# KdaiP/StableTTS

Hardware: AMD Instinct MI355X
Metric: mel-frames/sec (whole node), 31M DiT, n_timesteps=10+CFG (higher is better)
Workload: dtype f16

## Files before the change

stabletts_amd/csrc/attention.hip:

```cpp
#include "common.h"
#include "launch.h"

#if (defined(ST_ABL_NOEXP) || defined(ST_ABL_NOSUM)) && !defined(ST_DEVTOOLS)
#error "ST_ABL_* (ablation builds: results are garbage) need -DST_DEVTOOLS"
#endif
#ifdef ST_ABL_NOEXP
constexpr bool kAblNoExp = true;
#else
constexpr bool kAblNoExp = false;
#endif
#ifdef ST_ABL_NOSUM
constexpr bool kAblNoSum = true;
#else
constexpr bool kAblNoSum = false;
#endif
#ifndef ST_ATTN_WAVES
#define ST_ATTN_WAVES 8
#endif

namespace st {

template <class P, bool TRAIN, bool SPLIT = false, bool VLO = false>
__global__ __launch_bounds__(64 * ST_ATTN_WAVES, ST_ATTN_WAVES >= 16 || SPLIT ? 2 : 4) void attention_kernel(const AttnArgs a) {
    static_assert(!(TRAIN && SPLIT), "split-precision scores: inference kernel only");
    static_assert(!VLO || (TRAIN && !SPLIT), "hi + lo v: training kernel only");
    constexpr bool X3 = SPLIT || VLO;
    constexpr int NW = ST_ATTN_WAVES, QB = 32 * NW, QTILE = QB;
    using vec8 = typename P::vec8;
    constexpr int TILE_BYTES = 64 * 128;
    constexpr int NBUF = 3;
    constexpr int NT = X3 ? 3 : 2;
    constexpr int SMEM = NT * NBUF * TILE_BYTES > NW * 32 * 144 ? NT * NBUF * TILE_BYTES : NW * 32 * 144;
    __shared__ __attribute__((aligned(16))) unsigned char smem[SMEM];
    __shared__ float wave_lse[NW];
    unsigned char* Ks = smem;
    unsigned char* Vs = smem + NBUF * TILE_BYTES;
    unsigned char* KLs = smem + 2 * NBUF * TILE_BYTES;
    unsigned char* VLs = KLs;

    const int T = a.T, Tp = a.Tp, H = a.H;
    const int qtiles = (T + QB - 1) / QB;
    const int j = blockIdx.x >> 3;
    const int qt = j % qtiles, nh = (j / qtiles) * 8 + (blockIdx.x & 7);
    if (nh >= a.n_items * H) return;
    const int n = nh / H, h = nh % H;
    const int mb = n % a.mask_mod;
    if (a.t_lim && qt * QTILE >= a.t_lim[mb]) return;
    const int kvend = a.kv_end[mb];
    const int nfull = a.n_full[mb];
    const float* kbias = a.kbias + (size_t)mb * Tp;

    const int tid = threadIdx.x, lane = tid & 63;
    const int wave = __builtin_amdgcn_readfirstlane(tid >> 6);
    const int l31 = lane & 31, hi = lane >> 5;
    const int query = qt * QB + wave * 32 + l31;

    const unsigned char* qbase = (const unsigned char*)a.q + ((size_t)nh * T) * 128;
    const unsigned char* kbase = (const unsigned char*)a.k + ((size_t)nh * T) * 128;
    const unsigned char* vbase = (const unsigned char*)a.vt + ((size_t)nh * 64) * Tp * 2;
    const unsigned char* qlbase = SPLIT ? (const unsigned char*)a.q_lo + ((size_t)nh * T) * 128 : nullptr;
    const unsigned char* klbase = SPLIT ? (const unsigned char*)a.k_lo + ((size_t)nh * T) * 128 : nullptr;
    const unsigned char* vlbase = VLO ? (const unsigned char*)a.vt_lo + ((size_t)nh * 64) * Tp * 2 : nullptr;
    if constexpr (TRAIN) {
        if (qt * QB >= kvend) {
            if (query < T) {
                unsigned char* orow = (unsigned char*)a.out + (((size_t)n * T + query) * (H * 64) + h * 64) * 2 + hi * 64;
#pragma unroll
                for (int i = 0; i < 4; ++i) *(uint4*)(orow + 16 * i) = make_uint4(0, 0, 0, 0);
                if (hi == 0) a.lse[(size_t)nh * T + query] = 0.f;
            }
            return;
        }
    }

    vec8 qf[4];
#pragma unroll
    for (int ks = 0; ks < 4; ++ks) {
        uint4 v = make_uint4(0, 0, 0, 0);
        if (query < T) v = *(const uint4*)(qbase + (size_t)query * 128 + ks * 32 + hi * 16);
        qf[ks] = as_vec8<P>(v);
    }
    vec8 qlf[SPLIT ? 4 : 1];
    if constexpr (SPLIT) {
#pragma unroll
        for (int ks = 0; ks < 4; ++ks) {
            uint4 v = make_uint4(0, 0, 0, 0);
            if (query < T) v = *(const uint4*)(qlbase + (size_t)query * 128 + ks * 32 + hi * 16);
            qlf[ks] = as_vec8<P>(v);
        }
    }

    const int ntiles = (kvend + 63) >> 6;
    auto sgpr_ptr = [](const unsigned char* p) {
        const uintptr_t v = (uintptr_t)p;
        return (const unsigned char*)(((uintptr_t)(unsigned)__builtin_amdgcn_readfirstlane((int)(v >> 32)) << 32) |
                                      (unsigned)__builtin_amdgcn_readfirstlane((int)(unsigned)v));
    };
    auto issueKV = [&](int kt, int buf) {
        auto k_piece = [&](int piece) {
            int ln = lane;
            if constexpr (TRAIN) asm volatile("" : "+v"(ln));
            const int row = piece * 8 + (ln >> 3);
            const int seg = (ln & 7) ^ ((row >> 1) & 7);
            const int key = min(kt * 64 + row, T - 1);
            glds16s(sgpr_ptr(kbase), (unsigned)(key * 128 + seg * 16), Ks + buf * TILE_BYTES + piece * 1024);
            if constexpr (SPLIT) glds16s(sgpr_ptr(klbase), (unsigned)(key * 128 + seg * 16), KLs + buf * TILE_BYTES + piece * 1024);
        };
        auto v_piece = [&](int piece) {
            const int row = piece * 8 + (lane >> 3);
            const int seg = (lane & 7) ^ ((row >> 1) & 7);
            glds16s(sgpr_ptr(vbase + (size_t)kt * 128), (unsigned)((row * Tp + seg * 8) * 2), Vs + buf * TILE_BYTES + piece * 1024);
            if constexpr (VLO) glds16s(sgpr_ptr(vlbase + (size_t)kt * 128), (unsigned)((row * Tp + seg * 8) * 2), VLs + buf * TILE_BYTES + piece * 1024);
        };
        if constexpr (NW <= 8) {
#pragma unroll
            for (int k = 0; k < 8 / NW; ++k) { k_piece(wave * (8 / NW) + k); v_piece(wave * (8 / NW) + k); }
        } else {
            if (wave < 8) k_piece(wave); else v_piece(wave - 8);
        }
    };

    int row_off[2], swz[2];
#pragma unroll
    for (int b = 0; b < 2; ++b) {
        const int row = b * 32 + l31;
        row_off[b] = row * 128; swz[b] = (row >> 1) & 7;
    }

    f32x16_t o[2];
#pragma unroll
    for (int d = 0; d < 2; ++d)
#pragma unroll
        for (int r = 0; r < 16; ++r) o[d][r] = 0.f;
    constexpr float kBig = 8192.0f, kLazyTrain = 8.0f, kFloor = -20000.0f;
    unsigned drop_rh = 0;
    if constexpr (TRAIN) { if (a.drop.thresh16) drop_rh = a.drop.rowh[(size_t)nh * T + (query < T ? query : T - 1)]; }
    float m_ref = 0.f, l_run = 0.f;
    vec8 qaug, kaug;
#pragma unroll
    for (int i = 0; i < 8; ++i) { qaug[i] = to16<P>(0.f); kaug[i] = to16<P>(0.f); }
    if (hi == 0) kaug[0] = to16<P>(1.0f);

    if (ntiles > 0) issueKV(0, 0);
    if (ntiles > 1) { issueKV(1, 1); if constexpr (NW <= 8) { if constexpr (NW == 8) { if constexpr (X3) ST_DMA_WAIT(3); else ST_DMA_WAIT(2); } else { if constexpr (X3) ST_DMA_WAIT(6); else ST_DMA_WAIT(4); } } else ST_DMA_WAIT(1); }
    else ST_DMA_WAIT(0);
    __syncthreads();

    const int ntiles_run = ntiles;
    bool dead = false;
    if constexpr (!TRAIN) dead = a.t_lim && qt * QB + wave * 32 >= a.t_lim[mb];
    int buf = 0;
    for (int kt = 0; kt < ntiles_run; ++kt) {
        if (kt + 2 < ntiles_run) issueKV(kt + 2, buf >= 1 ? buf - 1 : NBUF - 1);
        if (!dead) {

        f32x16_t s[2];
        const bool partial = (kt + 1) * 64 > nfull;
        auto scores = [&]() __attribute__((always_inline)) {
#pragma unroll
            for (int kb = 0; kb < 2; ++kb) {
#pragma unroll
                for (int r = 0; r < 16; ++r) s[kb][r] = 0.f;
                s[kb] = P::mfma(kaug, qaug, s[kb]);
                const unsigned char* kp = Ks + buf * TILE_BYTES + row_off[kb];
#pragma unroll
                for (int ks = 0; ks < 4; ++ks) {
                    const vec8 kfrag = as_vec8<P>(*(const uint4*)(kp + (((ks * 2 + hi) ^ swz[kb]) << 4)));
                    s[kb] = P::mfma(kfrag, qf[ks], s[kb]);
                    if constexpr (SPLIT) {
                        s[kb] = P::mfma(kfrag, qlf[ks], s[kb]);
                        const unsigned char* klp = KLs + buf * TILE_BYTES + row_off[kb];
                        s[kb] = P::mfma(as_vec8<P>(*(const uint4*)(klp + (((ks * 2 + hi) ^ swz[kb]) << 4))), qf[ks], s[kb]);
                    }
                }
                __builtin_amdgcn_sched_barrier(0);
            }
            if (partial) {
#pragma unroll
                for (int kb = 0; kb < 2; ++kb)
#pragma unroll
                    for (int g4 = 0; g4 < 4; ++g4) {
                        const float4 bz = *(const float4*)(kbias + kt * 64 + kb * 32 + 8 * g4 + 4 * hi);
                        s[kb][4 * g4 + 0] += bz.x; s[kb][4 * g4 + 1] += bz.y;
                        s[kb][4 * g4 + 2] += bz.z; s[kb][4 * g4 + 3] += bz.w;
                    }
            }
        };
        vec8 pf[4];
        float psum[2];
        scores();
        if constexpr (TRAIN) {
            float mx = s[0][0];
#pragma unroll
            for (int kb = 0; kb < 2; ++kb)
#pragma unroll
                for (int r = 0; r < 16; ++r) mx = fmaxf(mx, s[kb][r]);
            mx = xor32_max(mx);
// ... 313 lines not shown
        }
    }
}

template <class P>
static hipError_t launch_attention_small(const AttnArgs& a, hipStream_t s) {
    static bool attr_done_dev[64] = {};
    int dev_ = 0;
    if (hipGetDevice(&dev_) != hipSuccess || dev_ < 0 || dev_ >= 64) return hipErrorInvalidDevice;
    if (!attr_done_dev[dev_]) {
        hipError_t e = hipFuncSetAttribute((const void*)attention_small_kernel<P>, hipFuncAttributeMaxDynamicSharedMemorySize, kAttnSmallLds);
        if (e != hipSuccess) return e;
        attr_done_dev[dev_] = true;
    }
    const int total = a.n_items * a.H * ((a.T + 31) / 32);
    const int grid = ((total + 7) / 8) * 8;
    hipLaunchKernelGGL((attention_small_kernel<P>), dim3(grid), dim3(512), kAttnSmallLds, s, a);
    return hipGetLastError();
}

hipError_t launch_attention(int dtype, const AttnArgs& a, hipStream_t s) {
    if (!a.zeros || !a.kbias) return hipErrorInvalidValue;
    const int qtiles = (a.T + 32 * ST_ATTN_WAVES - 1) / (32 * ST_ATTN_WAVES);
    const int total = a.n_items * a.H * qtiles;
    if (!a.lse && !a.q_lo && a.small_max_blocks > 0 && total <= a.small_max_blocks)
        return dtype == DT_BF16 ? launch_attention_small<OpBF16>(a, s) : launch_attention_small<OpF16>(a, s);
    const int grid = 8 * ((a.n_items * a.H + 7) / 8) * qtiles;
    if (a.lse) {
        if (a.vt_lo) {
            if (dtype == DT_BF16) hipLaunchKernelGGL((attention_kernel<OpBF16, true, false, true>), dim3(grid), dim3(64 * ST_ATTN_WAVES), 0, s, a);
            else                  hipLaunchKernelGGL((attention_kernel<OpF16, true, false, true>), dim3(grid), dim3(64 * ST_ATTN_WAVES), 0, s, a);
            return hipGetLastError();
        }
        if (dtype == DT_BF16) hipLaunchKernelGGL((attention_kernel<OpBF16, true>), dim3(grid), dim3(64 * ST_ATTN_WAVES), 0, s, a);
        else                  hipLaunchKernelGGL((attention_kernel<OpF16, true>), dim3(grid), dim3(64 * ST_ATTN_WAVES), 0, s, a);
        return hipGetLastError();
    }
    if (a.q_lo || a.k_lo) {
        if (!a.q_lo || !a.k_lo) return hipErrorInvalidValue;
        static bool attr_done_dev[64][2] = {};
        int dev_ = 0;
        if (hipGetDevice(&dev_) != hipSuccess || dev_ < 0 || dev_ >= 64) return hipErrorInvalidDevice;
        const int di = dtype == DT_BF16 ? 0 : 1;
        const void* fn = di == 0 ? (const void*)attention_kernel<OpBF16, false, true> : (const void*)attention_kernel<OpF16, false, true>;
        if (!attr_done_dev[dev_][di]) {
            hipError_t e = hipFuncSetAttribute(fn, hipFuncAttributeMaxDynamicSharedMemorySize, 0);
            (void)e;
            attr_done_dev[dev_][di] = true;
        }
        if (di == 0) hipLaunchKernelGGL((attention_kernel<OpBF16, false, true>), dim3(grid), dim3(64 * ST_ATTN_WAVES), 0, s, a);
        else         hipLaunchKernelGGL((attention_kernel<OpF16, false, true>), dim3(grid), dim3(64 * ST_ATTN_WAVES), 0, s, a);
        return hipGetLastError();
    }
    if (dtype == DT_BF16) hipLaunchKernelGGL((attention_kernel<OpBF16, false>), dim3(grid), dim3(64 * ST_ATTN_WAVES), 0, s, a);
    else                  hipLaunchKernelGGL((attention_kernel<OpF16, false>), dim3(grid), dim3(64 * ST_ATTN_WAVES), 0, s, a);
    return hipGetLastError();
}

}
```

stabletts_amd/csrc/engine.cpp:

```cpp
#include "engine_dit.h"
#include "train_launch.h"
#include "mas_launch.h"
#include "align_train_launch.h"

#include <algorithm>
#include <cmath>
#include <cstdio>
#include <cstring>
#include <map>
#include <string>
#include <vector>

using namespace st;
using namespace sthost;

namespace sthost {
std::string g_create_error;

const char* kProfNames[PC_COUNT] = {
    "prep", "prenet_conv", "in_proj", "film_ln1", "qkv_rope", "attention", "out_proj", "ln2",
    "ffn_conv1", "ffn_conv2", "lsc_conv", "final_proj", "ode_update", "train_forward", "train_backward"};

int dev_alloc(st_engine* e, void** p, size_t bytes) {
    HIPCHK(e, hipMalloc(p, bytes ? bytes : 16));
// ... 371 lines not shown
    };
    if (film) {
        ConvGemmArgs a = base_args(e, p, dit->inx, N);
        a.a0 = p.x16; a.c0 = dit->Mp; a.a0_mod = p.B; a.a1 = p.x16lo; a.c1 = dit->Mp; a.a1_mod = p.B; a.c2 = dit->Mp;
        a.bias = nullptr;
        a.add32 = p.cpart; a.add_clamp = p.B;
        a.out32 = p.X; a.out16 = p.skip16[0];
        fuse_ln1(a, 0);
        ProfScope ps(e, s, PC_INPROJ, conv_flops(p, dit->inx, N));
        HIPCHK(e, gemm(e, 1, EPI_F32, a, s));
    } else {
        FilmLnArgs a; memset(&a, 0, sizeof(a));
        a.X = p.X; a.h16 = p.h16; a.film = nullptr; a.film_mod = 1;
        a.ada = ada_of(0); a.ada_stride = 6 * C; a.shift_off = 0; a.scale_off = C;
        a.mask = mask; a.mask_mod = p.B; a.mask_out = 0; a.T = T; a.rows = N * T;
        ProfScope ps(e, s, PC_FILM_LN1, 0);
        HIPCHK(e, launch_film_ln(e->dt, a, s));
    }
    if (film && cap) capture(e, "h0", p.skip16[0], rowsC, true, s);
    for (int i = 0; i < L; ++i) {
        const std::string bn = "b" + std::to_string(i) + ".";
        const float* ada_i = ada_of(i);
        if (skips && i >= L / 2) {
            const int j = i - L / 2;
            ConvGemmArgs a = base_args(e, p, dit->lsc[j], N);
            a.a0 = p.cur16; a.c0 = C; a.a1 = p.skip16[L - 1 - i]; a.c1 = C;
            a.out32 = p.X;
            fuse_ln1(a, i);
            ProfScope ps(e, s, PC_LSC, conv_flops(p, dit->lsc[j], N));
            if (!(dit->skip_mask >> PC_LSC & 1)) HIPCHK(e, gemm(e, 3, EPI_F32, a, s));
        }
        if (cap) { capture(e, bn + "x1", p.X, rowsC, false, s); capture(e, bn + "h1", p.h16, rowsC, true, s); }
        {
            ConvGemmArgs a = base_args(e, p, dit->qkv[i], N);
            a.a0 = p.h16; a.c0 = C;
            a.q = p.q16; a.k = p.k16; a.vt = p.vt16; a.rope_cos = dit->rope_cos; a.rope_sin = dit->rope_sin;
            if (split_qk) { a.q_lo = p.q16lo; a.k_lo = p.k16lo; }
            a.Tp = p.Tp; a.n_heads = dit->H;
            if ((int)dit->qkv_frag.size() == L) a.w_frag = dit->qkv_frag[i];
            a.qscale = 1.4426950408889634f / sqrtf((float)(C / dit->H));
            ProfScope ps(e, s, PC_QKV, conv_flops(p, dit->qkv[i], N));
            if (!(dit->skip_mask >> PC_QKV & 1)) HIPCHK(e, gemm(e, 1, EPI_QKV, a, s));
        }
        if (cap) {
            capture(e, bn + "q", p.q16, rowsC, true, s); capture(e, bn + "k", p.k16, rowsC, true, s);
            capture(e, bn + "vt", p.vt16, (int64_t)N * C * p.Tp, true, s);
        }
        {
            AttnArgs a; memset(&a, 0, sizeof(a));
            a.q = p.q16; a.k = p.k16; a.vt = p.vt16; a.out = p.ao16; a.kbias = p.kbias; a.mask_mod = p.B; a.zeros = e->zeros;
            a.kv_end = p.kv_end; a.n_full = p.n_full; a.T = T; a.Tp = p.Tp; a.H = dit->H; a.n_items = N;
            a.small_max_blocks = dit->conc == 1 ? dit->attn_small_blocks : 0;
            if (split_qk) { a.q_lo = p.q16lo; a.k_lo = p.k16lo; }
            if (dec_fast_paths) a.lse_max = dit->lse_cells;
            if (ragged) a.t_lim = p.t_lim;
            ProfScope ps(e, s, PC_ATTN, 4.0 * (double)N * dit->H * (double)T * T * (C / dit->H));
            if (!(dit->skip_mask >> PC_ATTN & 1)) HIPCHK(e, launch_attention(e->dt, a, s));
        }
        if (cap) capture(e, bn + "attn", p.ao16, rowsC, true, s);
        const bool fused = dec_fast_paths && dit->fused_ffn && !cap && (int)dit->ffn_stream.size() == L && dit->ffn_stream[i] &&
                           (int64_t)dit->conc * N * ((T + kFfnFusedFrames - 1) / kFfnFusedFrames) >= e->tile.big_min_blocks;
        void* h2buf = fused ? p.h2_16 : p.h16;
        {
            ConvGemmArgs a = base_args(e, p, dit->oproj[i], N);
            a.a0 = p.ao16; a.c0 = C; a.mask = mask; a.gate = ada_i + 2 * C; a.gate_stride = 6 * C; a.out32 = p.X;
            a.ln_h16 = h2buf; a.ln_film = nullptr; a.ln_film_mod = 1;
            a.ln_ada = ada_i; a.ln_ada_stride = 6 * C; a.ln_shift_off = 3 * C; a.ln_scale_off = 4 * C; a.ln_mask_out = 1;
            if (dec_fast_paths && (int)dit->oproj_frag.size() == L && !cap) a.w_frag = dit->oproj_frag[i];
            ProfScope ps(e, s, PC_OPROJ, conv_flops(p, dit->oproj[i], N));
            if (!(dit->skip_mask >> PC_OPROJ & 1)) HIPCHK(e, gemm(e, 1, EPI_RESGATE, a, s));
        }
        if (cap) { capture(e, bn + "x2", p.X, rowsC, false, s); capture(e, bn + "h2", p.h16, rowsC, true, s); }
        if (!fused) {
            ConvGemmArgs a = base_args(e, p, dit->ffn1[i], N);
            a.a0 = p.h16; a.c0 = C; a.mask = mask; a.flags = GF_SILU | GF_MASK; a.out16 = p.u16;
            ProfScope ps(e, s, PC_FFN1, conv_flops(p, dit->ffn1[i], N));
            HIPCHK(e, gemm(e, 3, EPI_ACT16, a, s));
        }
        if (cap) capture(e, bn + "u", p.u16, (int64_t)N * T * F, true, s);
        void* copy16 = (skips && i + 1 < L / 2) ? p.skip16[i + 1] : p.cur16;
        {
            ConvGemmArgs a = base_args(e, p, dit->ffn2[i], N);
            a.a0 = p.u16; a.c0 = F; a.mask = mask; a.gate = ada_i + 5 * C; a.gate_stride = 6 * C; a.out32 = p.X;
            if (fused) { a.a0 = h2buf; a.c0 = C; a.w = dit->ffn_stream[i]; a.bias1 = dit->ffn1[i].bias; a.cmid = F; a.flags = GF_SILU | GF_MASK; }
            a.out16 = copy16;
            if (i + 1 == L) a.out16_lo = p.cur16lo;
            if (i + 1 < ln1_by_ffn) fuse_ln1(a, i + 1);
            else if (dec_fast_paths && !cap) a.out32_readonly = 1;
            ProfScope ps(e, s, PC_FFN2, conv_flops(p, dit->ffn2[i], N) + (fused ? conv_flops(p, dit->ffn1[i], N) : 0.0));
            if (dit->skip_mask >> PC_FFN2 & 1) {}
            else if (fused && dit->fused_ffn == 3) HIPCHK(e, launch_ffn_wino_f16(a, s));
            else if (fused) HIPCHK(e, e->dt == DT_BF16 ? launch_ffn_fused_bf16(a, s) : launch_ffn_fused_f16(a, s));
            else HIPCHK(e, gemm(e, 3, EPI_RESGATE, a, s));
        }
        if (cap) {
            if (film && i + 1 < ln1_by_ffn) capture(e, bn + "x3", copy16, rowsC, true, s);
            else capture(e, bn + "x3", p.X, rowsC, false, s);
        }
    }
    {
        ConvGemmArgs a = base_args(e, p, dit->fin, N);
        a.a0 = p.cur16; a.c0 = C; a.a1 = p.cur16lo; a.c1 = C; a.c2 = C; a.mask = mask; a.flags = GF_MASK; a.out32 = p.v32;
        ProfScope ps(e, s, PC_FINAL, conv_flops(p, dit->fin, N));
        HIPCHK(e, gemm(e, 1, EPI_F32, a, s));
    }
    if (cap) capture(e, "v", p.v32, (int64_t)N * T * dit->Mp, false, s);
// ... 566 lines not shown
    HIPCHK(e, hipStreamSynchronize((hipStream_t)stream));
    *nonfinite = *dit->status_host != 0;
    dit->arena_poisoned(e);
    return ST_OK;
}

int st_cfm_loss_prep(const float* x1, const float* z, const float* t_rand, float sigma_min, int B, int M, int T, float* t, float* y,
                     float* u, void* stream) {
    if (!x1 || !z || !t_rand || !t || !y || !u) return align_fail(ST_ERR_INVALID, "null tensor pointer");
    if (B < 1 || M < 1 || T < 1 || B > 65535) return align_fail(ST_ERR_INVALID, "shape out of range");
    if (launch_cfm_loss_prep(x1, z, t_rand, sigma_min, B, M, T, t, y, u, (hipStream_t)stream) != hipSuccess)
        return align_fail(ST_ERR_HIP, "cfm_loss_prep kernel launch failed");
    return ST_OK;
}

int st_cfm_loss(const float* pred, const float* u, const float* mask, int B, int M, int T, float* scratch, float* loss, void* stream) {
    if (!pred || !u || !mask || !scratch || !loss) return align_fail(ST_ERR_INVALID, "null tensor pointer");
    if (B < 1 || M < 1 || T < 1) return align_fail(ST_ERR_INVALID, "shape out of range");
    if (launch_cfm_loss(pred, u, mask, B, M, T, scratch, loss, (hipStream_t)stream) != hipSuccess)
        return align_fail(ST_ERR_HIP, "cfm_loss kernel launch failed");
    return ST_OK;
}

int st_cfm_loss_backward(const float* pred, const float* u, const float* scratch, const float* grad_loss, int B, int M, int T,
                         float* grad_pred, void* stream) {
    if (!pred || !u || !scratch || !grad_loss || !grad_pred) return align_fail(ST_ERR_INVALID, "null tensor pointer");
    if (B < 1 || M < 1 || T < 1) return align_fail(ST_ERR_INVALID, "shape out of range");
    if (launch_cfm_loss_bwd(pred, u, scratch, grad_loss, B, M, T, grad_pred, (hipStream_t)stream) != hipSuccess)
        return align_fail(ST_ERR_HIP, "cfm_loss_bwd kernel launch failed");
    return ST_OK;
}

int st_cfm_loss_scratch_floats(void) { return 2 * kCfmLossBlocks + 2; }

int st_last_solve_stats(const st_engine* e, int64_t* nfe, int64_t* steps, int64_t* rejects) {
    if (!e) return ST_ERR_INVALID;
    const DitState* dit = dit_or_null(e);
    if (nfe) *nfe = dit ? dit->last_nfe : 0;
    if (steps) *steps = dit ? dit->last_steps : 0;
    if (rejects) *rejects = dit ? dit->last_rejects : 0;
    return ST_OK;
}

int st_set_option(st_engine* e, const char* name, int value) {
    if (!e || !name) return ST_ERR_INVALID;
    const std::string n(name);
    if (n == "attention_precision") {
        if (value != 0 && value != 1) return e->fail(ST_ERR_INVALID, "attention_precision: 0 (16-bit q / k operands) or 1 (split hi + lo operands)");
        if (e->kind != KIND_DECODER) return e->fail(ST_ERR_UNSUPPORTED, "attention_precision: CFM decoder handles only");
        DitState* dit = dit_of(e);
        if (value != dit->attn_split) { dit->drop_graphs(); dit->attn_split = value; }
        return ST_OK;
    }
    if (n == "fused_ffn") return e->fail(ST_ERR_INVALID, "fused_ffn is read-only (ST_FUSED_FFN at st_create)");
    return e->fail(ST_ERR_INVALID, std::string("unknown option: ") + name);
}

int st_get_option(const st_engine* e, const char* name, int* value) {
    if (!e || !name || !value) return ST_ERR_INVALID;
    const DitState* dit = dit_or_null(e);
    const std::string n(name);
    if (n == "attention_precision") { *value = dit ? dit->attn_split : 0; return ST_OK; }
    if (n == "fused_ffn") { *value = dit ? dit->fused_ffn : -1; return ST_OK; }
    return ST_ERR_INVALID;
}

int st_attention_stats(st_engine* e, void* stream, float* max_lse) {
    if (!e || !max_lse) return ST_ERR_INVALID;
    DitState* dit = dit_or_null(e);
    if (!dit || !dit->lse_cells) return e->fail(ST_ERR_STATE, "attention statistics unavailable (allocation failed at st_create)");
    HIPCHK(e, hipSetDevice(e->device));
    HIPCHK(e, hipStreamSynchronize((hipStream_t)stream));
    int cells[kLseCells * 16];
    HIPCHK(e, hipMemcpy(cells, dit->lse_cells, sizeof(cells), hipMemcpyDeviceToHost));
    int best = (int)0x80000000;
    for (int c = 0; c < kLseCells; ++c) best = std::max(best, cells[c * 16]);
    HIPCHK(e, hipMemsetD32((hipDeviceptr_t)dit->lse_cells, (int)0x80000000, kLseCells * 16));
    if (best == (int)0x80000000) { *max_lse = -INFINITY; return ST_OK; }
    const int bits = best >= 0 ? best : best ^ 0x7fffffff;
    float v; memcpy(&v, &bits, 4);
    *max_lse = v * 0.6931471805599453f;
    return ST_OK;
}

int st_debug_capture(st_engine* e, int enable) {
    if (!e) return ST_ERR_INVALID;
    e->capture = enable != 0;
    if (!enable) {
        hipSetDevice(e->device);
        hipDeviceSynchronize();
        for (auto& kv : e->caps) if (kv.second.dev) hipFree(kv.second.dev);
        e->caps.clear();
    }
    return ST_OK;
}

int64_t st_debug_fetch(st_engine* e, const char* name, float* host_out, int64_t capacity) {
    if (!e || !name) return ST_ERR_INVALID;
    auto it = e->caps.find(name);
    if (it == e->caps.end() || !it->second.dev) { e->err = std::string("no captured tensor named ") + name; return ST_ERR_INVALID; }
    Captured& c = it->second;
    if (!host_out) return c.n;
    if (capacity < c.n) { e->err = "capacity too small"; return ST_ERR_INVALID; }
    if (hipSetDevice(e->device) != hipSuccess || hipDeviceSynchronize() != hipSuccess) return ST_ERR_HIP;
    if (!c.is16) {
        if (hipMemcpy(host_out, c.dev, (size_t)c.n * 4, hipMemcpyDeviceToHost) != hipSuccess) return ST_ERR_HIP;
        return c.n;
    }
    float* tmp = nullptr;
    if (hipMalloc((void**)&tmp, (size_t)c.n * 4) != hipSuccess) return ST_ERR_HIP;
    hipError_t r = launch_cvt16_to_f32(e->dt, c.dev, tmp, c.n, nullptr);
    if (r == hipSuccess) r = hipMemcpy(host_out, tmp, (size_t)c.n * 4, hipMemcpyDeviceToHost);
    hipFree(tmp);
    return r == hipSuccess ? c.n : (int64_t)ST_ERR_HIP;
}
// ... 47 lines not shown
```

stabletts_amd/csrc/engine_dit.h:

```cpp
#pragma once
#include "engine_internal.h"
#include "stream_fork.h"

constexpr int kMaxParts = 1 + sthost::StreamFork::kMaxChildren;
constexpr size_t kSplitKBytes = 32u << 20;

namespace sthost {

struct TrainState;

struct DitState : KindState {
    st_config cfg{};
    bool dec = true;
    int M = 0, Mp = 0, C = 0, F = 0, H = 0, L = 0, K = 0, G = 0;
    int n_vocab = 0;
    std::string blk(int i) const { return dec ? "blocks." + std::to_string(i) + ".block." : "encoder." + std::to_string(i) + "."; }
    struct PackList { std::vector<st::PackJob> jobs; st::PackJob* dev = nullptr; unsigned nblocks = 0; bool ready = false; bool recording = false; };
    PackList pk_fwd, pk_T;
    bool packed_once = false;

    std::vector<Conv> pre;
    Conv inx, inc, fin;
    std::vector<Conv> lsc, qkv, oproj, ffn1, ffn2;
    std::vector<void*> oproj_frag;
    std::vector<void*> qkv_frag;
    std::vector<void*> ffn_stream;

    float* rope_cos = nullptr; float* rope_sin = nullptr; int rope_T = 0;
    void* sink = nullptr;

    int64_t last_nfe = 0, last_steps = 0, last_rejects = 0;
    int* status_host = nullptr; int* status_dev = nullptr;
    bool arena_poisoned(st_engine* e) { if (status_host && *status_host) { *status_host = 0; e->ws_sig = 0; return true; } return false; }

    void* adams_buf = nullptr; size_t adams_bytes = 0;
    unsigned skip_mask = 0;
    int qkv_ws_min_tiles = 400;
    int qkv_ws = 1;
    int oproj_ws = 1;
    int oproj_ws_min_tiles = 1000;
    int qkv_rc1 = 1;
    int fused_ffn = -1;
    int attn_split = 0;
    unsigned* lse_cells = nullptr;
    int attn_small_blocks = 32;
    int conc = 1;
    StreamFork part_streams;

    struct SolveGraph {
        int B, T, n_steps, solver, use_cfg; float cfg_strength; const char* ws; int parts; int seen; hipGraphExec_t exec;
    };
    std::vector<SolveGraph> graphs;
    hipStream_t gstream = nullptr;
    void drop_graphs() {
        for (auto& g : graphs) if (g.exec) hipGraphExecDestroy(g.exec);
        graphs.clear();
    }

    TrainState* train = nullptr;

    ~DitState() override;
    int finalize(st_engine* e) override;
    int repack(st_engine* e, hipStream_t s) override;
    int64_t device_bytes() const override;
    int64_t train_serial() const override;
    void params_moved() override { pk_fwd.ready = false; pk_T.ready = false; drop_graphs(); }
    void arena_moved() override { drop_graphs(); }
};

inline DitState* dit_of(st_engine* e) { return state_of<DitState>(e); }
inline const DitState* dit_of(const st_engine* e) { return state_of<DitState>(e); }
inline const DitState* dit_or_null(const st_engine* e) { return e->kind == KIND_DECODER || e->kind == KIND_TEXT_ENCODER ? dit_of(e) : nullptr; }
inline DitState* dit_or_null(st_engine* e) { return const_cast<DitState*>(dit_or_null(const_cast<const st_engine*>(e))); }

int arena_fresh(st_engine* e, uint64_t sig, size_t used_bytes, hipStream_t s);
int ensure_rope(st_engine* e, int T, hipStream_t s);
int check_ready(st_engine* e, Kind kind, int B, int T);
int pack_all(st_engine* e, hipStream_t s);
bool pk_replay(st_engine* e, DitState::PackList& L, hipStream_t s, int* rc);
void pk_begin(DitState::PackList& L);
int pk_end(st_engine* e, DitState::PackList& L, hipStream_t s);
int pk_weight(st_engine* e, DitState::PackList& L, const float* src, int cout, int cin_total, int K, int ci_off, int ci_cnt, void* dst,
              int row_off, int cin_p, int col_off, int slice_w, int lo, hipStream_t s);
int pk_weight_t(st_engine* e, DitState::PackList& L, const float* src, int cout, int cin_total, int taps, int ci_off, int ci_cnt, void* dst,
                int cin_p, int ld, int col_off, hipStream_t s);
int pk_copy(st_engine* e, DitState::PackList& L, float* dst, const float* src, int n, hipStream_t s);

struct Plan {
    int B, T, Tp, N, Pn, n_t;
    bool cfg;
    void *mu16, *pre1, *pre2, *cond16, *cond16lo, *x16, *x16lo, *h16, *h2_16, *q16, *k16, *q16lo, *k16lo, *vt16, *ao16, *u16, *cur16, *cur16lo;
    void* skip16[8];
    float *cpart, *X, *v32, *xstate, *kbuf[7], *ynew, *ode_partial, *ode_out, *tvals, *emb, *th, *tau, *film, *cvec, *ada, *ada_tmp;
    int *n_full, *kv_end;
    int* t_lim;
    float* kbias;
    float* maskbuf;
// ... 18 lines not shown
```

stabletts_amd/csrc/launch.h:

```cpp
#pragma once
#include <hip/hip_runtime.h>
#include <stdint.h>

namespace st {

enum { DT_BF16 = 0, DT_F16 = 1 };

enum { EPI_ACT16 = 0, EPI_F32 = 1, EPI_RESGATE = 2, EPI_QKV = 3,
       EPI_GELU16 = 4,
       EPI_SILU = 5 };
enum { GF_SILU = 1, GF_MASK = 2,
       GF_K2_V_ONLY = 4 };

struct ConvGemmArgs {
    const void* a0; const void* a1;
    int c0, c1;
    int c2;
    int a0_mod, a1_mod;
    const void* w;
    long long w_item_stride;
    const float* bias;
    int cout, T, n_items;
    int tiles_f, tiles_c;
    const float* mask; int mask_mod;
// ... 11 lines not shown
    const float* rope_cos; const float* rope_sin;
    int Tp; float qscale; int n_heads;
    const void* zeros;
    const void* w_frag;
    void* sink;
    void* ln_h16;
    const float* ln_film; int ln_film_stride; int ln_film_mod;
    const float* ln_ada; int ln_ada_stride; int ln_shift_off; int ln_scale_off;
    int ln_mask_out;
    const int* t_lim; int t_lim_mod;
    void* act16; const void* dact16;
    unsigned long long drop_seed; unsigned drop_thresh16; float drop_scale;
    int ksplit;
    const float* bias1; int cmid;
    unsigned long long* dbg;
};

enum { G2_T128 = 0, G2_RC = 1, G2_K3PIPE = 2,
       G2_BIG = 3,
       G2_T64 = 4, G2_RC64 = 5,
       G2_PHASED = 6,
       G2_RC1 = 7 };
hipError_t launch_conv_gemm2_bf16(int cfg, int taps, int epi, const ConvGemmArgs& a, hipStream_t s);
hipError_t launch_conv_gemm2_f16(int cfg, int taps, int epi, const ConvGemmArgs& a, hipStream_t s);
hipError_t launch_splitk_finish_bf16(int epi, const ConvGemmArgs& a, const float* part, int S, hipStream_t s);
hipError_t launch_splitk_finish_f16(int epi, const ConvGemmArgs& a, const float* part, int S, hipStream_t s);
constexpr int kFfnFusedFrames = 126;
hipError_t launch_ffn_fused_bf16(const ConvGemmArgs& a, hipStream_t s);
hipError_t launch_ffn_fused_f16(const ConvGemmArgs& a, hipStream_t s);
hipError_t launch_pack_ffn_stream(int dtype, const float* src, int stage, int F, void* dst, hipStream_t s);
hipError_t launch_pack_ffn_wino(const float* src, int stage, int F, void* dst, hipStream_t s);
hipError_t launch_ffn_wino_f16(const ConvGemmArgs& a, hipStream_t s);
hipError_t launch_qkv_ws(int dtype, const ConvGemmArgs& a, hipStream_t s);
hipError_t launch_oproj_ws(int dtype, const ConvGemmArgs& a, hipStream_t s);
hipError_t launch_pack_qkv_frag(int dtype, const float* src, int plane, void* dst, hipStream_t s);
constexpr int kGemmFramesPerTile = 128;
constexpr int kGemmChannelsPerTile = 128;

struct DropCfg { unsigned long long seed; unsigned thresh16; float scale; const unsigned* rowh; const unsigned* colh; };

struct AttnArgs {
    const void* q; const void* k; const void* vt; void* out;
    const void* q_lo; const void* k_lo;
    const void* vt_lo;
    unsigned* lse_max;
    const float* kbias; int mask_mod;
    const int* kv_end; const int* n_full;
    int T, Tp, H, n_items;
    const void* zeros;
    float* lse;
    DropCfg drop;
    const int* t_lim;
    int small_max_blocks;
};
constexpr int kLseCells = 16;
hipError_t launch_attention(int dtype, const AttnArgs& a, hipStream_t s);

struct FilmLnArgs {
    float* X;
    void* h16;
    const float* film; int film_stride; int film_mod;
    const float* ada; int ada_stride;
    int shift_off, scale_off;
    const float* mask; int mask_mod;
    int mask_out;
    int T, rows;
};
hipError_t launch_film_ln(int dtype, const FilmLnArgs& a, hipStream_t s);

hipError_t launch_time_embed(const float* t, int n_t, int dim, float* emb, hipStream_t s);
hipError_t launch_silu_rows(const float* in, int64_t n, float* out, hipStream_t s);
struct LinearJobs { const float* in[8]; const float* W[8]; const float* bias[8]; float* out[8]; int n; };
hipError_t launch_linear_multi(const LinearJobs& J, int n, int k, int o, int silu_in, int silu_out, hipStream_t s);
hipError_t launch_linear(const float* in, int n, int k, const float* W, const float* bias, int o,
                         float* out, int silu_in, int silu_out, hipStream_t s);
constexpr int kFrameHalo = 4;
hipError_t launch_mask_prep(const float* mask, int B, int T, int Tp, int* n_full, int* kv_end, float* kbias, int* t_lim, hipStream_t s);

hipError_t launch_to_time_major(int dtype, const float* in, int B, int C, int T, int Cp,
                                float* out32, void* out16, void* out16lo, hipStream_t s);
hipError_t launch_from_time_major(const float* in, int B, int C, int T, int Cp, float* out, hipStream_t s, int* nonfinite = nullptr);
hipError_t launch_embed_tokens(const long long* tokens, const long long* lengths, const float* emb, int n_vocab,
                               int C, float scale, int B, int T, float* X, float* mask_out, hipStream_t s);
hipError_t launch_set_values(float* dst, const float* host_vals, int n, hipStream_t s);
hipError_t launch_delay(int us, hipStream_t s);
hipError_t launch_cvec_prep(const float* c, const float* fake_or_null, int B, int G, float* dst, hipStream_t s);
hipError_t launch_fill_rows16(int dtype, const float* vec, int C, int Cp, int T, void* out16, hipStream_t s);

hipError_t launch_cfg_combine(int dtype, const float* v, int B, int64_t per_item, int use_cfg, float s,
                              float* kout, float* xio, void* x16, void* x16lo, float dt, hipStream_t stream);
hipError_t launch_lincomb(int dtype, const float* x, const float* const* k, const float* coef, int nk,
                          int64_t n, float* y32, void* y16, void* y16lo, hipStream_t s);

hipError_t launch_pack_weight(int dtype, const float* src, int cout, int cin_total, int K, int ci_off,
                              int ci_cnt, void* dst, int row_off, int cin_p, int col_off, int slice_w, int lo,
                              hipStream_t s);
hipError_t launch_cvt16_to_f32(int dtype, const void* src, float* dst, int64_t n, hipStream_t s);
struct PackJob { const float* src; void* dst; int kind, cout, cin_total, K, ci_off, ci_cnt, row_off, cin_p, col_off, slice_w, lo; unsigned blk0; };
hipError_t launch_pack_jobs(int dtype, const PackJob* jobs_dev, int njobs, unsigned nblocks, hipStream_t s);

constexpr int kCfmLossBlocks = 1024;
hipError_t launch_cfm_loss_prep(const float* x1, const float* z, const float* t_rand, float sigma_min, int B, int M, int T,
                                float* t_out, float* y, float* u, hipStream_t s);
hipError_t launch_cfm_loss(const float* pred, const float* u, const float* mask, int B, int M, int T, float* scratch, float* loss, hipStream_t s);
hipError_t launch_cfm_loss_bwd(const float* pred, const float* u, const float* scratch, const float* grad_loss, int B, int M, int T, float* gpred, hipStream_t s);

// ... 17 lines not shown
```

Before: 1.364 million.

## Add opt-in 4-wave 64-query attention form interleaving softmax with MFMA

Adds a second inference attention kernel form in which each wave owns 64 queries as two 32-query halves. The score MFMAs of one half are interleaved with the exp and pack work of the other half, and with the PV MFMAs, so vector-ALU softmax work overlaps matrix-core work while K/V fragments loaded from LDS are shared by both halves. The form is selectable through a new `attention_form` engine option, which defaults to the existing 8-wave kernel. Separately, the existing kernel now issues the second K/V prefetch before forcing the Q registers to land. That part is on by default and only reorders when the Q load is waited on. The wide form raises register pressure and runs at lower occupancy.

```diff
diff --git a/stabletts_amd/csrc/attention.hip b/stabletts_amd/csrc/attention.hip
--- a/stabletts_amd/csrc/attention.hip
+++ b/stabletts_amd/csrc/attention.hip
@@ -18,12 +18,331 @@
 #define ST_ATTN_WAVES 8
 #endif
 
+#ifndef ST_ATTN_QWAIT
+#define ST_ATTN_QWAIT 3
+#endif
+
 namespace st {
 
-template <class P, bool TRAIN, bool SPLIT = false, bool VLO = false>
-__global__ __launch_bounds__(64 * ST_ATTN_WAVES, ST_ATTN_WAVES >= 16 || SPLIT ? 2 : 4) void attention_kernel(const AttnArgs a) {
+template <class V>
+__device__ __forceinline__ void q_landed(V (&qf)[4]) {
+    asm volatile("" : "+v"(qf[0]), "+v"(qf[1]), "+v"(qf[2]), "+v"(qf[3]));
+}
+
+template <class P>
+__device__ __forceinline__ void attention_wide_body(const AttnArgs& a, unsigned char* smem, float* wave_lse) {
+    constexpr int NW = 4, QB = 64 * NW, QTILE = QB;
+    using vec8 = typename P::vec8;
+    constexpr int TILE_BYTES = 64 * 128, NBUF = 3;
+    static_assert(2 * NBUF * TILE_BYTES >= NW * 64 * 144, "output staging lives in the ring");
+    unsigned char* Ks = smem;
+    unsigned char* Vs = smem + NBUF * TILE_BYTES;
+
+    const int T = a.T, Tp = a.Tp, H = a.H;
+    const int qtiles = (T + QB - 1) / QB;
+    const int j = blockIdx.x >> 3;
+    const int qt = j % qtiles, nh = (j / qtiles) * 8 + (blockIdx.x & 7);
+    if (nh >= a.n_items * H) return;
+    const int n = nh / H, h = nh % H;
+    const int mb = n % a.mask_mod;
+    if (a.t_lim && qt * QTILE >= a.t_lim[mb]) return;
+    const int kvend = a.kv_end[mb];
+    const int nfull = a.n_full[mb];
+    const float* kbias = a.kbias + (size_t)mb * Tp;
+
+    const int tid = threadIdx.x, lane = tid & 63;
+    const int wave = __builtin_amdgcn_readfirstlane(tid >> 6);
+    const int l31 = lane & 31, hi = lane >> 5;
+    const int q0 = qt * QB + wave * 64;
+
+    const unsigned char* qbase = (const unsigned char*)a.q + ((size_t)nh * T) * 128;
+    const unsigned char* kbase = (const unsigned char*)a.k + ((size_t)nh * T) * 128;
+    const unsigned char* vbase = (const unsigned char*)a.vt + ((size_t)nh * 64) * Tp * 2;
+
+    struct Half { vec8 qf[4]; vec8 qaug; f32x16_t o[2]; float m_ref, l_run; };
+    struct Tile { f32x16_t s[2]; unsigned pw[16]; float psum[2]; };
+    Half A, B;
+    auto init_half = [&](Half& x, int query) __attribute__((always_inline)) {
+#pragma unroll
+        for (int ks = 0; ks < 4; ++ks) {
+            uint4 v = make_uint4(0, 0, 0, 0);
+            if (query < T) v = *(const uint4*)(qbase + (size_t)query * 128 + ks * 32 + hi * 16);
+            x.qf[ks] = as_vec8<P>(v);
+        }
+#pragma unroll
+        for (int i = 0; i < 8; ++i) x.qaug[i] = to16<P>(0.f);
+#pragma unroll
+        for (int d = 0; d < 2; ++d)
+#pragma unroll
+            for (int r = 0; r < 16; ++r) x.o[d][r] = 0.f;
+        x.m_ref = 0.f; x.l_run = 0.f;
+    };
+    init_half(A, q0 + l31);
+    init_half(B, q0 + 32 + l31);
+    vec8 kaug;
+#pragma unroll
+    for (int i = 0; i < 8; ++i) kaug[i] = to16<P>(0.f);
+    if (hi == 0) kaug[0] = to16<P>(1.0f);
+
+    const int ntiles = (kvend + 63) >> 6;
+    auto sgpr_ptr = [](const unsigned char* p) {
+        const uintptr_t v = (uintptr_t)p;
+        return (const unsigned char*)(((uintptr_t)(unsigned)__builtin_amdgcn_readfirstlane((int)(v >> 32)) << 32) |
+                                      (unsigned)__builtin_amdgcn_readfirstlane((int)(unsigned)v));
+    };
+    auto issueKV = [&](int kt, int buf) {
+#pragma unroll
+        for (int k = 0; k < 2; ++k) {
+            const int piece = wave * 2 + k;
+            const int row = piece * 8 + (lane >> 3);
+            const int seg = (lane & 7) ^ ((row >> 1) & 7);
+            const int key = min(kt * 64 + row, T - 1);
+            glds16s(sgpr_ptr(kbase), (unsigned)(key * 128 + seg * 16), Ks + buf * TILE_BYTES + piece * 1024);
+            glds16s(sgpr_ptr(vbase + (size_t)kt * 128), (unsigned)((row * Tp + seg * 8) * 2), Vs + buf * TILE_BYTES + piece * 1024);
+        }
+    };
+    int row_off[2], swz[2];
+#pragma unroll
+    for (int b = 0; b < 2; ++b) {
+        const int row = b * 32 + l31;
+        row_off[b] = row * 128; swz[b] = (row >> 1) & 7;
+    }
+    constexpr float kBig = 8192.0f, kFloor = -20000.0f;
+
+    if (ntiles > 0) issueKV(0, 0);
+    if (ntiles > 1) issueKV(1, 1);
+#if ST_ATTN_QWAIT & 1
+    q_landed(A.qf); q_landed(B.qf);
+#endif
+    if (ntiles > 1) ST_DMA_WAIT(4);
+    else ST_DMA_WAIT(0);
+    __syncthreads();
+
+    bool deadA = false, deadB = false;
+    if (a.t_lim) { const int tl = a.t_lim[mb]; deadA = q0 >= tl; deadB = q0 + 32 >= tl; }
+    int buf = 0;
+    auto kfrag = [&](int kb, int ks) __attribute__((always_inline)) {
+        return as_vec8<P>(*(const uint4*)(Ks + buf * TILE_BYTES + row_off[kb] + (((ks * 2 + hi) ^ swz[kb]) << 4)));
+    };
+    auto vfrag = [&](int d, int g) __attribute__((always_inline)) {
+        return as_vec8<P>(*(const uint4*)(Vs + buf * TILE_BYTES + row_off[d] + (((g * 2 + hi) ^ swz[d]) << 4)));
+    };
+    auto bias = [&](Tile& t, int kt) __attribute__((always_inline)) {
+#pragma unroll
+        for (int kb = 0; kb < 2; ++kb)
+#pragma unroll
+            for (int g4 = 0; g4 < 4; ++g4) {
+                const float4 bz = *(const float4*)(kbias + kt * 64 + kb * 32 + 8 * g4 + 4 * hi);
+                t.s[kb][4 * g4 + 0] += bz.x; t.s[kb][4 * g4 + 1] += bz.y;
+                t.s[kb][4 * g4 + 2] += bz.z; t.s[kb][4 * g4 + 3] += bz.w;
+            }
+    };
+    auto scores = [&](Half& x, Tile& t, int kt) __attribute__((always_inline)) {
+#pragma unroll
+        for (int kb = 0; kb < 2; ++kb) {
+#pragma unroll
+            for (int r = 0; r < 16; ++r) t.s[kb][r] = 0.f;
+            t.s[kb] = P::mfma(kaug, x.qaug, t.s[kb]);
+#pragma unroll
+            for (int ks = 0; ks < 4; ++ks) t.s[kb] = P::mfma(kfrag(kb, ks), x.qf[ks], t.s[kb]);
+            __builtin_amdgcn_sched_barrier(0);
+        }
+        if ((kt + 1) * 64 > nfull) bias(t, kt);
+    };
+    auto raise = [&](Half& x, const Tile& t, bool first) __attribute__((always_inline)) {
+        float mx = t.s[0][0];
+#pragma unroll
+        for (int kb = 0; kb < 2; ++kb)
+#pragma unroll
+            for (int r = 0; r < 16; ++r) mx = fmaxf(mx, t.s[kb][r]);
+        mx = xor32_max(mx);
+        const bool need = first || mx > 0.0f;
+        const float m_new = need ? (float)to16<P>(fmaxf(x.m_ref + mx, kFloor)) : x.m_ref;
+        const float alpha = first ? 1.0f : __builtin_amdgcn_exp2f(x.m_ref - m_new);
+        x.l_run *= alpha;
+#pragma unroll
+        for (int d = 0; d < 2; ++d)
+#pragma unroll
+            for (int r = 0; r < 16; ++r) x.o[d][r] *= alpha;
+        x.m_ref = m_new;
+        if (hi == 0) x.qaug[0] = to16<P>(-x.m_ref);
+    };
+    auto pairs = [&](Tile& t, int p0, int p1) __attribute__((always_inline)) {
+#pragma unroll
+        for (int i = p0; i < p1; ++i) {
+            const int kb = i >> 3, r = (i & 7) * 2;
+            float e0, e1;
+            if constexpr (kAblNoExp) { e0 = t.s[kb][r] * 0.001f; e1 = t.s[kb][r + 1] * 0.001f; }
+            else { e0 = __builtin_amdgcn_exp2f(t.s[kb][r]); e1 = __builtin_amdgcn_exp2f(t.s[kb][r + 1]); }
+            if constexpr (!kAblNoSum) {
+                t.psum[0] = add_f32_scalar(t.psum[0], e0);
+                t.psum[1] = add_f32_scalar(t.psum[1], e1);
+            }
+            typedef __attribute__((ext_vector_type(2))) typename P::elem v2;
+            v2 w; w[0] = to16<P>(e0); w[1] = to16<P>(e1);
+            t.pw[i] = __builtin_bit_cast(unsigned, w);
+            asm volatile("" : "+v"(t.pw[i]), "+v"(t.psum[0]), "+v"(t.psum[1]));
+        }
+    };
+    auto pfrag = [&](const Tile& t, int g) __attribute__((always_inline)) {
+        return as_vec8<P>(make_uint4(t.pw[4 * g], t.pw[4 * g + 1], t.pw[4 * g + 2], t.pw[4 * g + 3]));
+    };
+    auto numerators = [&](Tile& t) __attribute__((always_inline)) { t.psum[0] = 0.f; t.psum[1] = 0.f; pairs(t, 0, 16); };
+    auto over = [&](const Tile& t, int kt) __attribute__((always_inline)) { return kt != 0 && __any(!(t.psum[0] + t.psum[1] <= kBig)); };
+    auto redo = [&](Half& x, Tile& t, int kt) __attribute__((always_inline)) {
+        scores(x, t, kt);
+        raise(x, t, false);
+        scores(x, t, kt);
+        numerators(t);
+    };
+    auto pv = [&](Half& x, const Tile& t) __attribute__((always_inline)) {
+#pragma unroll
+        for (int d = 0; d < 2; ++d)
+#pragma unroll
+            for (int g = 0; g < 4; ++g) x.o[d] = P::mfma(vfrag(d, g), pfrag(t, g), x.o[d]);
+    };
+    auto tile_end = [&](int kt) __attribute__((always_inline)) {
+        if (kt + 2 < ntiles) ST_DMA_WAIT(4);
+        else ST_DMA_WAIT(0);
+        __syncthreads();
+        buf = buf == NBUF - 1 ? 0 : buf + 1;
+    };
+
+    if (ntiles > 0) {
+        Tile t;
+        if (!deadA) { scores(A, t, 0); raise(A, t, true); }
+        if (!deadB) { scores(B, t, 0); raise(B, t, true); }
+    }
+
+    if (deadB) {
+        for (int kt = 0; kt < ntiles; ++kt) {
+            if (kt + 2 < ntiles) issueKV(kt + 2, buf >= 1 ? buf - 1 : NBUF - 1);
+            if (!deadA) {
+                Tile t;
+                scores(A, t, kt);
+                numerators(t);
+                if (over(t, kt)) redo(A, t, kt);
+                A.l_run += t.psum[0] + t.psum[1];
+                __builtin_amdgcn_sched_barrier(0);
+                pv(A, t);
+            }
+            tile_end(kt);
+        }
+    } else {
+        for (int kt = 0; kt < ntiles; ++kt) {
+            if (kt + 2 < ntiles) issueKV(kt + 2, buf >= 1 ? buf - 1 : NBUF - 1);
+            Tile tA, tB;
+            vec8 kf[2][4], vf[2][4];
+#pragma unroll
+            for (int kb = 0; kb < 2; ++kb)
+#pragma unroll
+                for (int ks = 0; ks < 4; ++ks) kf[kb][ks] = kfrag(kb, ks);
+#pragma unroll
+            for (int kb = 0; kb < 2; ++kb) {
+#pragma unroll
+                for (int r = 0; r < 16; ++r) tA.s[kb][r] = 0.f;
+                tA.s[kb] = P::mfma(kaug, A.qaug, tA.s[kb]);
+#pragma unroll
+                for (int ks = 0; ks < 4; ++ks) tA.s[kb] = P::mfma(kf[kb][ks], A.qf[ks], tA.s[kb]);
+                __builtin_amdgcn_sched_barrier(0);
+            }
+            if ((kt + 1) * 64 > nfull) bias(tA, kt);
+            tA.psum[0] = 0.f; tA.psum[1] = 0.f;
+#pragma unroll
+            for (int kb = 0; kb < 2; ++kb) {
+#pragma unroll
+                for (int r = 0; r < 16; ++r) tB.s[kb][r] = 0.f;
+                __builtin_amdgcn_sched_barrier(0);
+                tB.s[kb] = P::mfma(kaug, B.qaug, tB.s[kb]);
+                pairs(tA, kb * 8 + 0, kb * 8 + 2);
+                __builtin_amdgcn_sched_barrier(0);
+#pragma unroll
+                for (int ks = 0; ks < 4; ++ks) {
+                    tB.s[kb] = P::mfma(kf[kb][ks], B.qf[ks], tB.s[kb]);
+                    if (ks == 0) pairs(tA, kb * 8 + 2, kb * 8 + 4);
+                    if (ks == 1) pairs(tA, kb * 8 + 4, kb * 8 + 5);
+                    if (ks == 2) pairs(tA, kb * 8 + 5, kb * 8 + 7);
+                    if (ks == 3) pairs(tA, kb * 8 + 7, kb * 8 + 8);
+                    __builtin_amdgcn_sched_barrier(0);
+                }
+            }
+#pragma unroll
+            for (int d = 0; d < 2; ++d)
+#pragma unroll
+                for (int g = 0; g < 4; ++g) vf[d][g] = vfrag(d, g);
+            __builtin_amdgcn_sched_barrier(0);
+            if ((kt + 1) * 64 > nfull) bias(tB, kt);
+            if (over(tA, kt)) redo(A, tA, kt);
+            A.l_run += tA.psum[0] + tA.psum[1];
+            tB.psum[0] = 0.f; tB.psum[1] = 0.f;
+            __builtin_amdgcn_sched_barrier(0);
+#pragma unroll
+            for (int d = 0; d < 2; ++d)
+#pragma unroll
+                for (int g = 0; g < 4; ++g) {
+                    A.o[d] = P::mfma(vf[d][g], pfrag(tA, g), A.o[d]);
+                    pairs(tB, (d * 4 + g) * 2, (d * 4 + g) * 2 + 2);
+                    __builtin_amdgcn_sched_barrier(0);
+                }
+            if (over(tB, kt)) redo(B, tB, kt);
+            B.l_run += tB.psum[0] + tB.psum[1];
+            __builtin_amdgcn_sched_barrier(0);
+#pragma unroll
+            for (int d = 0; d < 2; ++d)
+#pragma unroll
+                for (int g = 0; g < 4; ++g) B.o[d] = P::mfma(vf[d][g], pfrag(tB, g), B.o[d]);
+            tile_end(kt);
+        }
+    }
+    const float ltA = xor32_sum(A.l_run), ltB = xor32_sum(B.l_run);
+    const float invA = ltA > 0.f ? 1.0f / ltA : 0.f, invB = ltB > 0.f ? 1.0f / ltB : 0.f;
+    if (a.lse_max) {
+        float v = -3.0e38f;
+        if (!deadA && q0 + l31 < T && q0 + l31 < kvend && ltA > 0.f) v = A.m_ref + log2f(ltA);
+        if (!deadB && q0 + 32 + l31 < T && q0 + 32 + l31 < kvend && ltB > 0.f) v = fmaxf(v, B.m_ref + log2f(ltB));
+#pragma unroll
+        for (int off = 16; off > 0; off >>= 1) v = fmaxf(v, __shfl_xor(v, off));
+        if (lane == 0) wave_lse[wave] = v;
+        __syncthreads();
+        if (tid == 0) {
+            float b = wave_lse[0];
+#pragma unroll
+            for (int w = 1; w < NW; ++w) b = fmaxf(b, wave_lse[w]);
+            int bits = __float_as_int(b);
+            bits = bits >= 0 ? bits : bits ^ 0x7fffffff;
+            atomicMax((int*)a.lse_max + ((blockIdx.x % kLseCells) << 4), bits);
+        }
+    }
+    if (deadA) return;
+    unsigned char* mine = smem + wave * (64 * 144);
+    auto park = [&](const Half& x, float inv, int hf) __attribute__((always_inline)) {
+#pragma unroll
+        for (int d = 0; d < 2; ++d)
+#pragma unroll
+            for (int q4 = 0; q4 < 4; ++q4)
+                *(uint2*)(mine + (hf * 32 + l31) * 144 + (d * 32 + 8 * q4 + 4 * hi) * 2) =
+                    pack4<P>(x.o[d][4 * q4 + 0] * inv, x.o[d][4 * q4 + 1] * inv, x.o[d][4 * q4 + 2] * inv, x.o[d][4 * q4 + 3] * inv);
+    };
+    park(A, invA, 0);
+    if (!deadB) park(B, invB, 1);
+    const int rsub = lane >> 3, seg = lane & 7;
+    unsigned char* obase = (unsigned char*)a.out + (((size_t)n * T + q0) * (H * 64) + h * 64) * 2 + seg * 16;
+    const int nrows = deadB ? 32 : 64;
+#pragma unroll
+    for (int i = 0; i < 8; ++i) {
+        const int row = i * 8 + rsub;
+        if (row < nrows) {
+            const uint4 v = *(const uint4*)(mine + row * 144 + seg * 16);
+            if (q0 + row < T) *(uint4*)(obase + (size_t)row * (H * 64) * 2) = v;
+        }
+    }
+}
+
+template <class P, bool TRAIN, bool SPLIT = false, bool VLO = false, int FORM = 0>
+__global__ __launch_bounds__(FORM ? 256 : 64 * ST_ATTN_WAVES, FORM ? 2 : (ST_ATTN_WAVES >= 16 || SPLIT ? 2 : 4)) void attention_kernel(const AttnArgs a) {
     static_assert(!(TRAIN && SPLIT), "split-precision scores: inference kernel only");
     static_assert(!VLO || (TRAIN && !SPLIT), "hi + lo v: training kernel only");
+    static_assert(FORM == 0 || (FORM == 1 && !TRAIN && !SPLIT && !VLO && ST_ATTN_WAVES == 8), "form 1: the 16-bit inference kernel, 256-query blocks");
     constexpr bool X3 = SPLIT || VLO;
     constexpr int NW = ST_ATTN_WAVES, QB = 32 * NW, QTILE = QB;
     using vec8 = typename P::vec8;
@@ -37,6 +356,7 @@
     unsigned char* Vs = smem + NBUF * TILE_BYTES;
     unsigned char* KLs = smem + 2 * NBUF * TILE_BYTES;
     unsigned char* VLs = KLs;
+    if constexpr (FORM == 1) { attention_wide_body<P>(a, smem, wave_lse); return; }
 
     const int T = a.T, Tp = a.Tp, H = a.H;
     const int qtiles = (T + QB - 1) / QB;
@@ -142,7 +462,13 @@
     if (hi == 0) kaug[0] = to16<P>(1.0f);
 
     if (ntiles > 0) issueKV(0, 0);
-    if (ntiles > 1) { issueKV(1, 1); if constexpr (NW <= 8) { if constexpr (NW == 8) { if constexpr (X3) ST_DMA_WAIT(3); else ST_DMA_WAIT(2); } else { if constexpr (X3) ST_DMA_WAIT(6); else ST_DMA_WAIT(4); } } else ST_DMA_WAIT(1); }
+#if ST_ATTN_QWAIT & 2
+    if constexpr (!TRAIN && !X3) { if (ntiles > 1) issueKV(1, 1); q_landed(qf); }
+    if (ntiles > 1) { if constexpr (TRAIN || X3) issueKV(1, 1); if constexpr (NW <= 8) {
+#else
+    if (ntiles > 1) { issueKV(1, 1); if constexpr (NW <= 8) {
+#endif
+        if constexpr (NW == 8) { if constexpr (X3) ST_DMA_WAIT(3); else ST_DMA_WAIT(2); } else { if constexpr (X3) ST_DMA_WAIT(6); else ST_DMA_WAIT(4); } } else ST_DMA_WAIT(1); }
     else ST_DMA_WAIT(0);
     __syncthreads();
 
@@ -562,6 +888,16 @@
         else         hipLaunchKernelGGL((attention_kernel<OpF16, false, true>), dim3(grid), dim3(64 * ST_ATTN_WAVES), 0, s, a);
         return hipGetLastError();
     }
+    if (a.form == 1) {
+#if ST_ATTN_WAVES == 8
+        if (dtype == DT_BF16) hipLaunchKernelGGL((attention_kernel<OpBF16, false, false, false, 1>), dim3(grid), dim3(256), 0, s, a);
+        else                  hipLaunchKernelGGL((attention_kernel<OpF16, false, false, false, 1>), dim3(grid), dim3(256), 0, s, a);
+        return hipGetLastError();
+#else
+        return hipErrorInvalidValue;
+#endif
+    }
+    if (a.form != 0) return hipErrorInvalidValue;
     if (dtype == DT_BF16) hipLaunchKernelGGL((attention_kernel<OpBF16, false>), dim3(grid), dim3(64 * ST_ATTN_WAVES), 0, s, a);
     else                  hipLaunchKernelGGL((attention_kernel<OpF16, false>), dim3(grid), dim3(64 * ST_ATTN_WAVES), 0, s, a);
     return hipGetLastError();
diff --git a/stabletts_amd/csrc/engine.cpp b/stabletts_amd/csrc/engine.cpp
--- a/stabletts_amd/csrc/engine.cpp
+++ b/stabletts_amd/csrc/engine.cpp
@@ -447,6 +447,7 @@
             a.kv_end = p.kv_end; a.n_full = p.n_full; a.T = T; a.Tp = p.Tp; a.H = dit->H; a.n_items = N;
             a.small_max_blocks = dit->conc == 1 ? dit->attn_small_blocks : 0;
             if (split_qk) { a.q_lo = p.q16lo; a.k_lo = p.k16lo; }
+            else a.form = dit->attn_form;
             if (dec_fast_paths) a.lse_max = dit->lse_cells;
             if (ragged) a.t_lim = p.t_lim;
             ProfScope ps(e, s, PC_ATTN, 4.0 * (double)N * dit->H * (double)T * T * (C / dit->H));
@@ -1119,6 +1120,13 @@
         if (value != dit->attn_split) { dit->drop_graphs(); dit->attn_split = value; }
         return ST_OK;
     }
+    if (n == "attention_form") {
+        if (value != 0 && value != 1) return e->fail(ST_ERR_INVALID, "attention_form: 0 (8 waves x 32 queries) or 1 (4 waves x 64 queries)");
+        if (e->kind != KIND_DECODER) return e->fail(ST_ERR_UNSUPPORTED, "attention_form: CFM decoder handles only");
+        DitState* dit = dit_of(e);
+        if (value != dit->attn_form) { dit->drop_graphs(); dit->attn_form = value; }
+        return ST_OK;
+    }
     if (n == "fused_ffn") return e->fail(ST_ERR_INVALID, "fused_ffn is read-only (ST_FUSED_FFN at st_create)");
     return e->fail(ST_ERR_INVALID, std::string("unknown option: ") + name);
 }
@@ -1128,6 +1136,7 @@
     const DitState* dit = dit_or_null(e);
     const std::string n(name);
     if (n == "attention_precision") { *value = dit ? dit->attn_split : 0; return ST_OK; }
+    if (n == "attention_form") { *value = dit ? dit->attn_form : 0; return ST_OK; }
     if (n == "fused_ffn") { *value = dit ? dit->fused_ffn : -1; return ST_OK; }
     return ST_ERR_INVALID;
 }
diff --git a/stabletts_amd/csrc/engine_dit.h b/stabletts_amd/csrc/engine_dit.h
--- a/stabletts_amd/csrc/engine_dit.h
+++ b/stabletts_amd/csrc/engine_dit.h
@@ -43,6 +43,7 @@
     int fused_ffn = -1;
     int attn_split = 0;
     unsigned* lse_cells = nullptr;
+    int attn_form = 0;
     int attn_small_blocks = 32;
     int conc = 1;
     StreamFork part_streams;
diff --git a/stabletts_amd/csrc/launch.h b/stabletts_amd/csrc/launch.h
--- a/stabletts_amd/csrc/launch.h
+++ b/stabletts_amd/csrc/launch.h
@@ -87,6 +87,7 @@
     DropCfg drop;
     const int* t_lim;
     int small_max_blocks;
+    int form;
 };
 constexpr int kLseCells = 16;
 hipError_t launch_attention(int dtype, const AttnArgs& a, hipStream_t s);
```

New measurement: 1.374 million (median of 6 runs). No clear change (+0.7%).
